# SHI-Labs/Prompt-Free-Diffusion

Measured on AMD Instinct MI355X. Metric: images/sec @512x512 50-step DDIM, SD-v1.5+SeeCoder, higher is better.
Workload: dtype f16; 1 GPU; [c2] SD-v1.5 UNet + seecoder-v1-0, 512x512, 50-step DDIM (50 real steps), CFG 2.0, fp16, batch=4/GPU, 1 SeeCoder encode(s) + VAE decode per batch; global_batch=4, parallelism=dp1, world_size_reported_by_backend=1, collectives_forced_at_world_1=False

## Files before the change

prompt-free-diffusion_amd/csrc/gemm_glds.hip:

```cpp
#include <type_traits>

#include <stdlib.h>

#include "pfd_common.h"

int pfd_ln_rowstats_launch(const half_t* x, long ldx, int M, int C, float* out, hipStream_t s, bool prof);

namespace {

constexpr int BK = 64;
constexpr int BN = 160;
constexpr int ROWB = BK * 2;

__device__ __attribute__((aligned(256))) half_t g_zero_page[128];

struct G160Params {
  const half_t* A;
  const half_t* W;
  const half_t* bias;
  const half_t* rowvec;
  const half_t* R;
  half_t* C;
  float* ws;
  half_t* Ct;
// ... 1021 lines not shown
#pragma nounroll
      for (int ky = 0; ky < 3; ++ky) {
#pragma nounroll
        for (int kx = 0; kx < 3; ++kx) {
          const int tap = ky * 3 + kx;
          if (tap < 8) issue_w(stage ^ 1, tap + 1, cb);
          else if (cb + 1 < cb_end) issue_w(stage ^ 1, 0, cb + 1);
          if (cb + 1 < cb_end && tap < P_SLOTS) issue_patch_slot(pbuf ^ 1, cb + 1, tap);
          const char* wt = smem + OFF_W + stage * WT_BYTES;
#pragma unroll
          for (int ks = 0; ks < 2; ++ks) {
            half8_t af[WMB], bf[5];
#pragma unroll
            for (int i = 0; i < WMB; ++i) {
              const int r = rbase[i] + toff;
              af[i] = *reinterpret_cast<const half8_t*>(patch + r * ROWB + ((((ks * 4 + g) + (r & ~1)) & 7) << 4));
            }
            const int bo = ks ? boff1 : boff0;
#pragma unroll
            for (int j = 0; j < 5; ++j) bf[j] = *reinterpret_cast<const half8_t*>(wt + bo + j * 16 * ROWB);
#pragma unroll
            for (int i = 0; i < WMB; ++i)
#pragma unroll
              for (int j = 0; j < 5; ++j)
                acc[i][j] = __builtin_amdgcn_mfma_f32_16x16x32_f16(bf[j], af[i], acc[i][j], 0, 0, 0);
          }
          __syncthreads();
          stage ^= 1;
          toff += 1;
        }
        toff += PW - 3;
      }
    }
  }
  epilogue160<WMB, 5, 512, false, true>(acc, p, lane, m0, n0, wm, wn, split, smem, tid, nullptr, tile_m * (256 / GN_SLAB));
}

template <int GN, int NWS = 2>
__global__ __launch_bounds__(768) void conv3x3_patch_ws_kernel(const G160Params p) {
  constexpr int NCW = 8, NLW = 4, WMB = 4;
  constexpr int PATCH_BYTES = PATCH_ROWS * ROWB;
  constexpr int WT_BYTES = BN * ROWB;
  constexpr int OFF_W = 2 * PATCH_BYTES;
  constexpr int SMEM = OFF_W + NWS * WT_BYTES;
  static_assert(NWS == 2 || (NWS == 3 && GN == 0), "the 3-stage weight ring serves the plain form");
  static_assert(SMEM <= 160 * 1024, "LDS");
  constexpr int P_INSTR = PATCH_ROWS / 8;
  __shared__ __attribute__((aligned(1024))) char smem[SMEM];
  PFD_ARG_BATCH_CONV(p);

  const int tid = threadIdx.x;
  const int lane = tid & 63;
  const int wave = __builtin_amdgcn_readfirstlane(tid >> 6);
  const int nblk = p.tiles_m * p.tiles_n;
  const int t = xcd_remap(blockIdx.x, nblk);
  const int tile_m = p.nmajor ? t % p.tiles_m : t / p.tiles_n;
  const int tile_n = p.nmajor ? t / p.tiles_m : t - tile_m * p.tiles_n;
  const int n0 = tile_n * BN;
  const int split = blockIdx.z;
  const int ncb = p.Cin / BK;
  const int cb_begin = split * p.kt_per_split;
  const int cb_end = min(ncb, cb_begin + p.kt_per_split);
  const int W = p.Wd, H = p.H;
  const int hw = H * W;
  const int TW = p.pt_w ? p.pt_w : W;
  const int TH = 256 / TW, PW = TW + 2;
  const int tpi = hw / 256, ntx = W / TW;
  const int b = tile_m / tpi;
  const int ti = tile_m - b * tpi;
  const int y0 = (ti / ntx) * TH, x0 = (ti % ntx) * TW;
  const int m0 = b * hw + y0 * W + x0;
  const int ncbs = max(0, cb_end - cb_begin);
  const int nsteps = ncbs * 9;
  auto cbv = [&](int i) -> int { return cb_begin + i; };

  auto block_barrier = [&]() {
    __builtin_amdgcn_sched_barrier(0);
    asm volatile("" ::: "memory");
    __builtin_amdgcn_s_barrier();
    asm volatile("" ::: "memory");
    __builtin_amdgcn_sched_barrier(0);
  };

  if (wave >= NCW) {
    const int lw = wave - NCW;
    const int srow = lane >> 3, cpos = lane & 7;
    const int prow_count = (TH + 2) * PW;
    const half_t* img = p.A + (long)b * hw * p.lda;
    auto piece_off = [&](int q) -> int {
      const int r = q * 8 + srow;
      const int py = r / PW, px = r - py * PW;
      const int y = y0 - 1 + py, x = x0 - 1 + px;
      const int c = (cpos - (r & ~1)) & 7;
      const bool ok = q < P_INSTR && r < prow_count && y >= 0 && y < H && x >= 0 && x < W;
      return ok ? (int)((y * W + x) * p.lda + c * 8) : -1;
    };
    int off_a[9], off_b[9];
#pragma unroll
    for (int tp = 0; tp < 9; ++tp) {
      off_a[tp] = piece_off(6 * tp + lw);
      off_b[tp] = piece_off(6 * tp + 4 + lw);
    }
    auto issue_patch = [&](int buf, int cb, int q, int off) {
      glds16(off >= 0 ? (const void*)(img + off + cb * BK) : (const void*)g_zero_page,
             smem + buf * PATCH_BYTES + q * 1024);
    };
    const half_t* wp[5];
#pragma unroll
    for (int j = 0; j < 5; ++j) {
      const int r = (lw + NLW * j) * 8 + srow;
      const int c = cpos ^ ((r >> 1) & 7);
      wp[j] = PFD_W_ROW_PTR(BN, p, tile_n, n0, r, c * 8);
    }
    auto issue_w = [&](int stage, int tap, int cb) {
      const long k0 = (long)(tap * (p.Cin / BK) + cb) * p.w_kstep;
#pragma unroll
      for (int j = 0; j < 5; ++j) glds16(wp[j] + k0, smem + OFF_W + stage * WT_BYTES + (lw + NLW * j) * 1024);
    };
    if constexpr (GN != 0) {
      const int c8 = ((cpos - (srow & ~1)) & 7) * 8;
      const float* tab = p.gn_table + (long)b * 2 * p.Cin + c8;
      const half_t* img2 = p.A2 + (long)b * hw * p.lda2;
      auto piece_pix = [&](int q) -> int {
        const int r = q * 8 + srow;
        const int py = r / PW, px = r - py * PW;
        const int y = y0 - 1 + py, x = x0 - 1 + px;
        const bool ok = q < P_INSTR && r < prow_count && y >= 0 && y < H && x >= 0 && x < W;
        return ok ? y * W + x : -1;
      };
      int pix_a[9], pix_b[9];
#pragma unroll
      for (int tp = 0; tp < 9; ++tp) {
        pix_a[tp] = piece_pix(6 * tp + lw);
        pix_b[tp] = piece_pix(6 * tp + 4 + lw);
      }
      float4_t sc[2], sh[2];
      auto load_tab = [&](int cb) {
#pragma unroll
        for (int j = 0; j < 2; ++j) {
          sc[j] = *reinterpret_cast<const float4_t*>(tab + cb * BK + 4 * j);
          sh[j] = *reinterpret_cast<const float4_t*>(tab + p.Cin + cb * BK + 4 * j);
        }
      };
      auto xform = [&](uint4 raw, bool ok) -> uint4 {
        Pack16 in, out;
        in.u = raw;
#pragma unroll
        for (int e = 0; e < 8; ++e) {
          float v = (float)in.e[e] * sc[e >> 2][e & 3] + sh[e >> 2][e & 3];
          if constexpr (GN == 2) v = pfd_silu(v);
          out.e[e] = (half_t)v;
        }
        return ok ? out.u : make_uint4(0, 0, 0, 0);
      };
      auto put = [&](int buf, int q, uint4 v) {
        lds_store16_opaque(smem + buf * PATCH_BYTES + q * 1024 + lane * 16, v);
      };
      auto fetch = [&](int cb, int pix) -> uint4 {
        const int ch = cb * BK;
        const int px = pix < 0 ? 0 : pix;
        const half_t* src = ch < p.gn_c1 ? img + (long)px * p.lda + (ch + c8)
                                         : img2 + (long)px * p.lda2 + (ch - p.gn_c1 + c8);
        return *reinterpret_cast<const uint4*>(src);
      };
      uint4 ra = make_uint4(0, 0, 0, 0), rb = ra;
      if (nsteps > 0) {
        issue_w(0, 0, cbv(0));
        load_tab(cbv(0));
        {
          uint4 fa[9], fb[9];
#pragma unroll
          for (int tp = 0; tp < 9; ++tp) {
            fa[tp] = fetch(cbv(0), pix_a[tp]);
            fb[tp] = lw < 2 ? fetch(cbv(0), pix_b[tp]) : make_uint4(0, 0, 0, 0);
          }
#pragma unroll
          for (int tp = 0; tp < 9; ++tp) {
            if (6 * tp + lw < P_INSTR) put(0, 6 * tp + lw, xform(fa[tp], pix_a[tp] >= 0));
            if (lw < 2 && 6 * tp + 4 + lw < P_INSTR) put(0, 6 * tp + 4 + lw, xform(fb[tp], pix_b[tp] >= 0));
          }
        }
        if (1 < ncbs) {
          load_tab(cbv(1));
          ra = fetch(cbv(1), pix_a[0]);
          if (lw < 2) rb = fetch(cbv(1), pix_b[0]);
        }
      }
      int stage = 0;
      for (int ci = 0; ci < ncbs; ++ci) {
        const int cb = cbv(ci);
        const int pbuf = ci & 1;
        const bool more = ci + 1 < ncbs;
        const int cb1 = more ? cbv(ci + 1) : cb, cb2 = ci + 2 < ncbs ? cbv(ci + 2) : cb;
#pragma unroll
        for (int tap = 0; tap < 9; ++tap) {
          __builtin_amdgcn_s_waitcnt(0x0070);
          block_barrier();
          if (tap < 8) issue_w(stage ^ 1, tap + 1, cb);
          else if (more) issue_w(stage ^ 1, 0, cb1);
          if (more) {
            uint4 na = ra, nb = rb;
            if (tap < 8) {
              na = fetch(cb1, pix_a[tap + 1]);
              if (lw < 2) nb = fetch(cb1, pix_b[tap + 1]);
            } else if (ci + 2 < ncbs) {
              na = fetch(cb2, pix_a[0]);
              if (lw < 2) nb = fetch(cb2, pix_b[0]);
            }
            const uint4 va = xform(ra, pix_a[tap] >= 0);
            uint4 vb = make_uint4(0, 0, 0, 0);
            if (lw < 2) vb = xform(rb, pix_b[tap] >= 0);
            if (tap == 8 && ci + 2 < ncbs) load_tab(cb2);
            if (6 * tap + lw < P_INSTR) put(pbuf ^ 1, 6 * tap + lw, va);
            if (lw < 2 && 6 * tap + 4 + lw < P_INSTR) put(pbuf ^ 1, 6 * tap + 4 + lw, vb);
            ra = na;
            rb = nb;
          }
          stage ^= 1;
        }
      }
    } else if constexpr (NWS == 3) {
      int off_p[14], q_p[14];
#pragma unroll
      for (int sl = 0; sl < 14; ++sl) {
        int q = 4 * sl + lw;
        if (q >= P_INSTR) q -= 8;
        q_p[sl] = q;
        off_p[sl] = piece_off(q);
      }
      if (nsteps > 0) {
#pragma unroll
        for (int sl = 0; sl < 14; ++sl)
          if (4 * sl + lw < P_INSTR) issue_patch(0, cbv(0), q_p[sl], off_p[sl]);
        issue_w(0, 0, cbv(0));
        issue_w(1, 1, cbv(0));
      }
      for (int ci = 0; ci < ncbs; ++ci) {
        const int cb = cbv(ci);
        const int pbuf = ci & 1;
        const bool more = ci + 1 < ncbs;
        const int cb1 = more ? cbv(ci + 1) : cb;
#pragma unroll
        for (int tap = 0; tap < 9; ++tap) {
          if (more) {
            if (tap == 0) __builtin_amdgcn_s_waitcnt(0x0F70 | 5);
            else if (tap == 1 || tap == 8) __builtin_amdgcn_s_waitcnt(0x0F70 | 7);
            else __builtin_amdgcn_s_waitcnt(0x0F70 | 9);
          } else {
            if (tap <= 7) __builtin_amdgcn_s_waitcnt(0x0F70 | 5);
            else __builtin_amdgcn_s_waitcnt(0x0F70);
          }
          block_barrier();
          if (tap + 2 < 9) issue_w((tap + 2) % 3, tap + 2, cb);
          else if (more) issue_w((tap + 2) % 3, tap + 2 - 9, cb1);
          if (more && tap <= 6) {
            issue_patch(pbuf ^ 1, cb1, q_p[2 * tap], off_p[2 * tap]);
            issue_patch(pbuf ^ 1, cb1, q_p[2 * tap + 1], off_p[2 * tap + 1]);
          }
        }
      }
    } else {
      if (nsteps > 0) {
#pragma unroll
        for (int tp = 0; tp < 9; ++tp) {
          if (6 * tp + lw < P_INSTR) issue_patch(0, cbv(0), 6 * tp + lw, off_a[tp]);
          if (lw < 2 && 6 * tp + 4 + lw < P_INSTR) issue_patch(0, cbv(0), 6 * tp + 4 + lw, off_b[tp]);
        }
        issue_w(0, 0, cbv(0));
      }
      int stage = 0;
      for (int ci = 0; ci < ncbs; ++ci) {
        const int cb = cbv(ci);
        const int pbuf = ci & 1;
        const bool more = ci + 1 < ncbs;
        const int cb1 = more ? cbv(ci + 1) : cb;
#pragma unroll
        for (int tap = 0; tap < 9; ++tap) {
          __builtin_amdgcn_s_waitcnt(0x0F70);
          block_barrier();
          if (tap < 8) issue_w(stage ^ 1, tap + 1, cb);
          else if (more) issue_w(stage ^ 1, 0, cb1);
          if (more) {
            if (6 * tap + lw < P_INSTR) issue_patch(pbuf ^ 1, cb1, 6 * tap + lw, off_a[tap]);
            if (lw < 2 && 6 * tap + 4 + lw < P_INSTR) issue_patch(pbuf ^ 1, cb1, 6 * tap + 4 + lw, off_b[tap]);
          }
          stage ^= 1;
        }
      }
    }
    block_barrier();
    block_barrier();
  } else {
    const int wm = wave >> 1, wn = wave & 1;
    const int l15 = lane & 15, g = lane >> 4;
    int rbase[WMB];
#pragma unroll
    for (int i = 0; i < WMB; ++i) {
      const int ql = wm * 64 + i * 16;
      const int ty = ql / TW, tx = ql - ty * TW;
      rbase[i] = ty * PW + tx + l15;
    }
    const int sw = (l15 >> 1) & 7;
    const int boff0 = wn * 80 * ROWB + l15 * ROWB + (((0 + g) ^ sw) << 4);
    const int boff1 = wn * 80 * ROWB + l15 * ROWB + (((4 + g) ^ sw) << 4);
    float4_t acc[WMB][5];
#pragma unroll
    for (int i = 0; i < WMB; ++i)
#pragma unroll
      for (int j = 0; j < 5; ++j) acc[i][j] = (float4_t){0.f, 0.f, 0.f, 0.f};
    auto a_off = [&](int i, int toff, int ks) -> int {
      const int r = rbase[i] + toff;
      return r * ROWB + ((((ks * 4 + g) + (r & ~1)) & 7) << 4);
    };
    {
      int stage = 0;
      for (int ci = 0; ci < ncbs; ++ci) {
        const char* patch = smem + (ci & 1) * PATCH_BYTES;
        int toff = 0;
#pragma nounroll
        for (int ky = 0; ky < 3; ++ky) {
#pragma nounroll
          for (int kx = 0; kx < 3; ++kx) {
            block_barrier();
            const char* wt = smem + OFF_W + stage * WT_BYTES;
#pragma unroll
            for (int ks = 0; ks < 2; ++ks) {
              half8_t af[WMB], bf[5];
#pragma unroll
              for (int i = 0; i < WMB; ++i) af[i] = *reinterpret_cast<const half8_t*>(patch + a_off(i, toff, ks));
              const int bo = ks ? boff1 : boff0;
#pragma unroll
              for (int j = 0; j < 5; ++j) bf[j] = *reinterpret_cast<const half8_t*>(wt + bo + j * 16 * ROWB);
#pragma unroll
              for (int i = 0; i < WMB; ++i)
#pragma unroll
                for (int j = 0; j < 5; ++j)
                  acc[i][j] = __builtin_amdgcn_mfma_f32_16x16x32_f16(bf[j], af[i], acc[i][j], 0, 0, 0);
            }
            if constexpr (NWS == 2) stage ^= 1;
            else if (++stage == NWS) stage = 0;
            toff += 1;
          }
          toff += PW - 3;
        }
      }
      block_barrier();
    }
    {
      const G160Params pe = reload_params();
      epilogue_stage<WMB, 5, true>(acc, pe, lane, m0, n0, wm, wn, split, smem);
    }
    asm volatile("s_waitcnt lgkmcnt(0)" ::: "memory");
    block_barrier();
  }
  const G160Params pe = reload_params();
  epilogue_store<256, 5, 768, false, true>(pe, m0, n0, smem, tid, tile_m * (256 / GN_SLAB));
}


__global__ __launch_bounds__(256) void splitk_reduce_kernel(const G160Params p) {
  const int nv = p.N / 8;
  const long nvec = (long)p.M * nv;
  for (long i = (long)blockIdx.x * 256 + threadIdx.x; i < nvec; i += (long)gridDim.x * 256) {
    const int m = (int)(i / nv);
    const int n = (int)(i - (long)m * nv) * 8;
    Pack16 bb, rv, rr;
    bb.u = *reinterpret_cast<const uint4*>(p.bias ? p.bias + n : g_zero_page);
    rv.u = *reinterpret_cast<const uint4*>(p.rowvec ? p.rowvec + (long)(m / p.rows_per_rv) * p.ldrv + n : g_zero_page);
    rr.u = *reinterpret_cast<const uint4*>(p.R ? p.R + res_row(p, m) * p.ldr + n : g_zero_page);
    float v[8] = {0, 0, 0, 0, 0, 0, 0, 0};
    for (int s0 = 0; s0 < p.splits; s0 += 4) {
      Pack16 a[4];
#pragma unroll
      for (int u = 0; u < 4; ++u)
        a[u].u = *reinterpret_cast<const uint4*>(reinterpret_cast<const half_t*>(p.ws) +
                                                 ((long)min(s0 + u, p.splits - 1) * p.M + m) * p.N + n);
#pragma unroll
      for (int u = 0; u < 4; ++u) {
        const float w = s0 + u < p.splits ? 1.f : 0.f;
#pragma unroll
        for (int e = 0; e < 8; ++e) v[e] += (float)a[u].e[e] * w;
      }
    }
    if (p.ln_in) {
      const float2* src = p.ln_in + (long)m * p.ln_P;
      float sum = 0.f, sq = 0.f;
#pragma unroll
      for (int j = 0; j < 8; ++j) {
        const float2 t = src[min(j, p.ln_P - 1)];
        const float w = j < p.ln_P ? 1.f : 0.f;
        sum = fmaf(t.x, w, sum);
        sq = fmaf(t.y, w, sq);
      }
      const float inv_k = 1.0f / (float)p.K;
      const float mean = sum * inv_k;
      const float rstd = rsqrtf(fmaxf(fmaf(-mean, mean, sq * inv_k), 0.f) + p.ln_eps);
      const float4_t c0 = *reinterpret_cast<const float4_t*>(p.ln_cs + n);
      const float4_t c1 = *reinterpret_cast<const float4_t*>(p.ln_cs + n + 4);
#pragma unroll
      for (int e = 0; e < 4; ++e) {
        v[e] = fmaf(v[e], rstd, -rstd * mean * c0[e]);
        v[4 + e] = fmaf(v[4 + e], rstd, -rstd * mean * c1[e]);
      }
    }
    Pack16 o;
#pragma unroll
    for (int e = 0; e < 8; ++e) {
      float x = v[e] + (float)bb.e[e];
      x += (float)rv.e[e];
      if (p.act == PFD_ACT_GELU) x = pfd_gelu(x);
      else if (p.act == PFD_ACT_RELU) x = fmaxf(x, 0.f);
      else if (p.act == PFD_ACT_SILU) x = pfd_silu(x);
      o.e[e] = (half_t)(x + (float)rr.e[e]);
    }
    *reinterpret_cast<uint4*>(p.C + (long)m * p.ldc + n) = o.u;
  }
}

constexpr int RGN_T = 256;
__global__ __launch_bounds__(RGN_T) void splitk_reduce_gn_kernel(const G160Params p) {
  constexpr int RW = RGN_T / 64, ROWS_SW = 3 * RW;
  __shared__ __attribute__((aligned(16))) float red[(RW + 1) * 320];
  const int tid = threadIdx.x, lane = tid & 63, w = tid >> 6;
  const int tiles_n = p.N / 160;
  const int slab = blockIdx.x / tiles_n, tile_n = blockIdx.x - slab * tiles_n;
  const int n = tile_n * 160 + (lane % 20) * 8;
  const bool active = lane < 60;
  const int rsub = lane / 20;
  float cs[8], cq[8];
#pragma unroll
  for (int e = 0; e < 8; ++e) cs[e] = cq[e] = 0.f;
  Pack16 bb;
  bb.u = *reinterpret_cast<const uint4*>(p.bias ? p.bias + n : g_zero_page);
  constexpr int SWEEPS = (GN_SLAB + ROWS_SW - 1) / ROWS_SW, U = SWEEPS < 3 ? SWEEPS : 3;
  static_assert(SWEEPS % U == 0, "sweeps in groups of U");
  for (int it0 = 0; it0 < SWEEPS; it0 += U) {
    int m[U];
    bool ok[U];
    Pack16 rv[U], rr[U];
    float v[U][8];
#pragma unroll
    for (int u = 0; u < U; ++u) {
      const int row_u = w * 3 + rsub + (it0 + u) * ROWS_SW;
      m[u] = min(slab * GN_SLAB + min(row_u, GN_SLAB - 1), p.M - 1);
      ok[u] = active && row_u < GN_SLAB && slab * GN_SLAB + row_u < p.M;
      rv[u].u = *reinterpret_cast<const uint4*>(p.rowvec ? p.rowvec + (long)(m[u] / p.rows_per_rv) * p.ldrv + n : g_zero_page);
      rr[u].u = *reinterpret_cast<const uint4*>(p.R ? p.R + res_row(p, m[u]) * p.ldr + n : g_zero_page);
#pragma unroll
      for (int e = 0; e < 8; ++e) v[u][e] = 0.f;
    }
    for (int s0 = 0; s0 < p.splits; s0 += 4) {
      Pack16 a[U][4];
#pragma unroll
      for (int u = 0; u < U; ++u)
#pragma unroll
        for (int k = 0; k < 4; ++k)
          a[u][k].u = *reinterpret_cast<const uint4*>(reinterpret_cast<const half_t*>(p.ws) +
                                                      ((long)min(s0 + k, p.splits - 1) * p.M + m[u]) * p.N + n);
#pragma unroll
      for (int u = 0; u < U; ++u)
#pragma unroll
        for (int k = 0; k < 4; ++k) {
          const float wgt = s0 + k < p.splits ? 1.f : 0.f;
#pragma unroll
          for (int e = 0; e < 8; ++e) v[u][e] += (float)a[u][k].e[e] * wgt;
        }
    }
#pragma unroll
    for (int u = 0; u < U; ++u) {
      Pack16 o;
      const float mk = ok[u] ? 1.f : 0.f;
#pragma unroll
      for (int e = 0; e < 8; ++e) {
        float x = v[u][e] + (float)bb.e[e];
        x += (float)rv[u].e[e];
        if (p.act == PFD_ACT_GELU) x = pfd_gelu(x);
        else if (p.act == PFD_ACT_RELU) x = fmaxf(x, 0.f);
        else if (p.act == PFD_ACT_SILU) x = pfd_silu(x);
        o.e[e] = (half_t)(x + (float)rr[u].e[e]);
        const float f = (float)o.e[e] * mk;
        cs[e] += f;
        cq[e] = fmaf(f, f, cq[e]);
      }
      if (ok[u]) *reinterpret_cast<uint4*>(p.C + (long)m[u] * p.ldc + n) = o.u;
    }
  }
  gn_slab_reduce<1, RGN_T>(cs, cq, tid, p.N / 32, slab, p.M / GN_SLAB, tiles_n, tile_n, p.gn_out, [&](int) { return red; });
}


struct GnFuse {
  const half_t* gamma;
  const half_t* beta;
  half_t* y;
  long ldy;
  float eps;
  int act, rows, skip_raw;
};
#ifndef PFD_GN_THREADS
#define PFD_GN_THREADS 1024
#endif
constexpr int GNF_T = PFD_GN_THREADS;
constexpr int GNF_MAX = 8192 / GNF_T;
constexpr int GNF_U = 2;

__global__ __launch_bounds__(GNF_T) void splitk_reduce_gnorm_kernel(const G160Params p, const GnFuse f) {
  __shared__ float red[2 * GNF_T / 64];
  __shared__ float gam_s[256], bet_s[256];
  const int cpg = p.N / 32, cpr = cpg / 4;
  const int lin = xcd_remap(blockIdx.x, gridDim.x);
  const int g = lin & 31, b = lin >> 5, tid = threadIdx.x, lane = tid & 63, wave = tid >> 6;
  const int HW = f.rows, total = HW * cpr;
  const int n_g = g * cpg;
  const long m_b = (long)b * HW;
  const int dr = GNF_T / cpr, dc = GNF_T - dr * cpr;
  const half_t* rvb = p.rowvec ? p.rowvec + (m_b / p.rows_per_rv) * p.ldrv + n_g : g_zero_page;
  const int rv_step = p.rowvec ? 4 : 0, b_step = p.bias ? 4 : 0;
  const half_t* bb0 = p.bias ? p.bias + n_g : g_zero_page;
  const long r_ld = p.R ? p.ldr : 0;
  const int r_step = p.R ? 4 : 0;
  const half_t* rb = p.R ? p.R + m_b * p.ldr + n_g : g_zero_page;
  uint2 v[GNF_MAX];
  int r = tid / cpr, ch = tid - r * cpr;
#pragma unroll
  for (int k0 = 0; k0 < GNF_MAX; k0 += GNF_U) {
    if (GNF_T * k0 >= total) {
#pragma unroll
      for (int u = 0; u < GNF_U; ++u) v[k0 + u] = make_uint2(0, 0);
      continue;
    }
    int ru[GNF_U], cu[GNF_U];
    bool on[GNF_U];
#pragma unroll
    for (int u = 0; u < GNF_U; ++u) {
      on[u] = tid + GNF_T * (k0 + u) < total;
      ru[u] = on[u] ? r : 0;
      cu[u] = on[u] ? ch : 0;
      r += dr;
      ch += dc;
      if (ch >= cpr) {
        ch -= cpr;
        ++r;
      }
    }
    Pack8 bq[GNF_U], rq[GNF_U], xq[GNF_U];
#pragma unroll
    for (int u = 0; u < GNF_U; ++u) {
      bq[u].u = *reinterpret_cast<const uint2*>(bb0 + cu[u] * b_step);
      rq[u].u = *reinterpret_cast<const uint2*>(rvb + cu[u] * rv_step);
      xq[u].u = *reinterpret_cast<const uint2*>(rb + (long)ru[u] * r_ld + cu[u] * r_step);
    }
    float acc[GNF_U][4];
#pragma unroll
    for (int u = 0; u < GNF_U; ++u)
#pragma unroll
      for (int e = 0; e < 4; ++e) acc[u][e] = 0.f;
    for (int s0 = 0; s0 < p.splits; s0 += 4) {
      Pack8 a[GNF_U][4];
#pragma unroll
      for (int u = 0; u < GNF_U; ++u)
#pragma unroll
        for (int q = 0; q < 4; ++q)
          a[u][q].u = *reinterpret_cast<const uint2*>(reinterpret_cast<const half_t*>(p.ws) +
                                                      ((long)min(s0 + q, p.splits - 1) * p.M + m_b + ru[u]) * p.N + n_g + cu[u] * 4);
#pragma unroll
      for (int q = 0; q < 4; ++q) {
        const float w = s0 + q < p.splits ? 1.f : 0.f;
#pragma unroll
        for (int u = 0; u < GNF_U; ++u)
#pragma unroll
          for (int e = 0; e < 4; ++e) acc[u][e] += (float)a[u][q].e[e] * w;
      }
    }
#pragma unroll
    for (int u = 0; u < GNF_U; ++u) {
      Pack8 o;
#pragma unroll
      for (int e = 0; e < 4; ++e) {
        float x = acc[u][e] + (float)bq[u].e[e];
        x += (float)rq[u].e[e];
        if (p.act == PFD_ACT_GELU) x = pfd_gelu(x);
        else if (p.act == PFD_ACT_RELU) x = fmaxf(x, 0.f);
        else if (p.act == PFD_ACT_SILU) x = pfd_silu(x);
        o.e[e] = (half_t)(x + (float)xq[u].e[e]);
      }
      if (on[u] && !f.skip_raw) *reinterpret_cast<uint2*>(p.C + (m_b + ru[u]) * p.ldc + n_g + cu[u] * 4) = o.u;
      v[k0 + u] = on[u] ? o.u : make_uint2(0, 0);
    }
  }
  if (tid < cpg) {
    gam_s[tid] = (float)f.gamma[n_g + tid];
    bet_s[tid] = (float)f.beta[n_g + tid];
  }
  float sm = 0.f, sq = 0.f;
#pragma unroll
  for (int k = 0; k < GNF_MAX; ++k) {
    Pack8 q;
    q.u = v[k];
#pragma unroll
    for (int e = 0; e < 4; ++e) {
      const float x = (float)q.e[e];
      sm += x;
      sq += x * x;
    }
  }
  sm = wave_sum(sm);
  sq = wave_sum(sq);
  constexpr int NWV = GNF_T / 64;
  if (lane == 0) {
    red[wave] = sm;
    red[NWV + wave] = sq;
  }
  __syncthreads();
  const float count = (float)HW * (float)cpg;
  float ts = red[0], tq = red[NWV];
#pragma unroll
  for (int w = 1; w < NWV; ++w) {
    ts += red[w];
    tq += red[NWV + w];
  }
  const float mean = ts / count;
  const float rstd = rsqrtf(fmaxf(tq / count - mean * mean, 0.f) + f.eps);
  half_t* yb = f.y + m_b * f.ldy + n_g;
  r = tid / cpr;
  ch = tid - r * cpr;
  asm volatile("" : "+v"(r), "+v"(ch));
#pragma unroll
  for (int k = 0; k < GNF_MAX; ++k) {
    if (tid + GNF_T * k < total) {
      Pack8 q, o;
      q.u = v[k];
#pragma unroll
      for (int e = 0; e < 4; ++e) {
        const float w = rstd * gam_s[ch * 4 + e];
        float t = (float)q.e[e] * w + (bet_s[ch * 4 + e] - mean * w);
        if (f.act == PFD_ACT_SILU) t = pfd_silu(t);
        o.e[e] = (half_t)t;
      }
      *reinterpret_cast<uint2*>(yb + (long)r * f.ldy + ch * 4) = o.u;
    }
    r += dr;
    ch += dc;
    if (ch >= cpr) {
      ch -= cpr;
      ++r;
    }
  }
// ... 332 lines not shown
```

Baseline: 8.101 images/s.

## Software-pipeline LDS fragment loads with MFMA in implicit-GEMM conv tap loop

Restructures the 3x3 conv tap loop in the LDS-resident implicit GEMM so A and B fragment loads for the second k-slice and the next tap are interleaved with MFMA columns, using sched_barrier fences to pin the order. The 9 taps are flattened into a loop of 8 prefetching steps plus a final one, and the block barrier moves to after each tap's compute so the next tap's A fragments are preloaded. The aim is to hide LDS read latency behind MFMA issue. The cost is higher register pressure from double-buffered A fragments and scheduling that is rigid and hand-tuned.

```diff
diff --git a/prompt-free-diffusion_amd/csrc/gemm_glds.hip b/prompt-free-diffusion_amd/csrc/gemm_glds.hip
--- a/prompt-free-diffusion_amd/csrc/gemm_glds.hip
+++ b/prompt-free-diffusion_amd/csrc/gemm_glds.hip
@@ -1347,47 +1347,103 @@
     }
     const int sw = (l15 >> 1) & 7;
     const int boff0 = wn * 80 * ROWB + l15 * ROWB + (((0 + g) ^ sw) << 4);
-    const int boff1 = wn * 80 * ROWB + l15 * ROWB + (((4 + g) ^ sw) << 4);
     float4_t acc[WMB][5];
 #pragma unroll
     for (int i = 0; i < WMB; ++i)
 #pragma unroll
       for (int j = 0; j < 5; ++j) acc[i][j] = (float4_t){0.f, 0.f, 0.f, 0.f};
-    auto a_off = [&](int i, int toff, int ks) -> int {
+    auto a_off = [&](int i, int toff) -> int {
       const int r = rbase[i] + toff;
-      return r * ROWB + ((((ks * 4 + g) + (r & ~1)) & 7) << 4);
+      return r * ROWB + (((g + (r & ~1)) & 7) << 4);
     };
     {
       int stage = 0;
+      half8_t a0[WMB], a1[WMB], bf[5];
+      int ao[WMB];
+      auto fence = [] { __builtin_amdgcn_sched_barrier(0); };
+      auto tap_step = [&](auto prefetch, const char* patch, const char* wt, int ntoff) {
+        auto lda = [&](int off) { return *reinterpret_cast<const half8_t*>(patch + off); };
+        auto ldb = [&](int j, int ks) { return *reinterpret_cast<const half8_t*>(wt + (boff0 ^ (ks << 6)) + j * 16 * ROWB); };
+        auto col = [&](const half8_t(&af)[WMB], int j) {
+#pragma unroll
+          for (int i = 0; i < WMB; ++i) acc[i][j] = __builtin_amdgcn_mfma_f32_16x16x32_f16(bf[j], af[i], acc[i][j], 0, 0, 0);
+        };
+        bf[1] = ldb(1, 0);
+        bf[0] = ldb(0, 0);
+        bf[2] = ldb(2, 0);
+        bf[3] = ldb(3, 0);
+        bf[4] = ldb(4, 0);
+        fence();
+        col(a0, 0);
+        fence();
+        a1[0] = lda(ao[0] ^ 64);
+        a1[1] = lda(ao[1] ^ 64);
+        bf[0] = ldb(0, 1);
+        fence();
+        col(a0, 1);
+        fence();
+        a1[2] = lda(ao[2] ^ 64);
+        a1[3] = lda(ao[3] ^ 64);
+        bf[1] = ldb(1, 1);
+        fence();
+        col(a0, 2);
+        fence();
+        bf[2] = ldb(2, 1);
+        fence();
+        col(a0, 3);
+        fence();
+        bf[3] = ldb(3, 1);
+        fence();
+        col(a0, 4);
+        if constexpr (decltype(prefetch)::value) {
+#pragma unroll
+          for (int i = 0; i < WMB; ++i) ao[i] = a_off(i, ntoff);
+        }
+        fence();
+        bf[4] = ldb(4, 1);
+        fence();
+        col(a1, 0);
+        fence();
+        if constexpr (decltype(prefetch)::value) {
+          a0[0] = lda(ao[0]);
+          a0[1] = lda(ao[1]);
+          fence();
+        }
+        col(a1, 1);
+        fence();
+        if constexpr (decltype(prefetch)::value) {
+          a0[2] = lda(ao[2]);
+          a0[3] = lda(ao[3]);
+          fence();
+        }
+        col(a1, 2);
+        col(a1, 3);
+        col(a1, 4);
+      };
+      auto next_stage = [&]() {
+        if constexpr (NWS == 2) stage ^= 1;
+        else if (++stage == NWS) stage = 0;
+      };
       for (int ci = 0; ci < ncbs; ++ci) {
         const char* patch = smem + (ci & 1) * PATCH_BYTES;
-        int toff = 0;
+        int toff = 0, kx = 0;
+        block_barrier();
+#pragma unroll
+        for (int i = 0; i < WMB; ++i) {
+          ao[i] = a_off(i, 0);
+          a0[i] = *reinterpret_cast<const half8_t*>(patch + ao[i]);
+        }
 #pragma nounroll
-        for (int ky = 0; ky < 3; ++ky) {
-#pragma nounroll
-          for (int kx = 0; kx < 3; ++kx) {
-            block_barrier();
-            const char* wt = smem + OFF_W + stage * WT_BYTES;
-#pragma unroll
-            for (int ks = 0; ks < 2; ++ks) {
-              half8_t af[WMB], bf[5];
-#pragma unroll
-              for (int i = 0; i < WMB; ++i) af[i] = *reinterpret_cast<const half8_t*>(patch + a_off(i, toff, ks));
-              const int bo = ks ? boff1 : boff0;
-#pragma unroll
-              for (int j = 0; j < 5; ++j) bf[j] = *reinterpret_cast<const half8_t*>(wt + bo + j * 16 * ROWB);
-#pragma unroll
-              for (int i = 0; i < WMB; ++i)
-#pragma unroll
-                for (int j = 0; j < 5; ++j)
-                  acc[i][j] = __builtin_amdgcn_mfma_f32_16x16x32_f16(bf[j], af[i], acc[i][j], 0, 0, 0);
-            }
-            if constexpr (NWS == 2) stage ^= 1;
-            else if (++stage == NWS) stage = 0;
-            toff += 1;
-          }
-          toff += PW - 3;
-        }
+        for (int tap = 0; tap < 8; ++tap) {
+          const int ntoff = toff + (kx == 2 ? PW - 2 : 1);
+          kx = kx == 2 ? 0 : kx + 1;
+          tap_step(std::true_type{}, patch, smem + OFF_W + stage * WT_BYTES, ntoff);
+          toff = ntoff;
+          next_stage();
+          block_barrier();
+        }
+        tap_step(std::false_type{}, patch, smem + OFF_W + stage * WT_BYTES, 0);
+        next_stage();
       }
       block_barrier();
     }
```

Result: faster. 8.208 images/s (median of 6 runs) (+1.3%).
